# Viictor/vrenderer

Hardware: AMD Instinct MI355X
Metric: shaded Gpixels/s at 8K terrain (higher is better)
Workload: dtype f32

## Files before the change

### vrenderer_amd/csrc/vr_internal.h

```cpp
#pragma once

#include <hip/hip_runtime.h>
#include <hip/hip_ext.h>
#include <stdint.h>
#include <stdlib.h>
#include <string>
#include <vector>

#include "../../include/vrterrain.h"

void vr_set_error(const char* fmt, ...);
#define VR_HIP(expr)                                                                  \
    do {                                                                              \
        hipError_t e__ = (expr);                                                      \
        if (e__ != hipSuccess) {                                                      \
            vr_set_error("%s:%d: %s -> %s", __FILE__, __LINE__, #expr, hipGetErrorString(e__)); \
            return e__ == hipErrorOutOfMemory ? VR_ERR_OUT_OF_MEMORY : VR_ERR_HIP;    \
        }                                                                             \
    } while (0)
#define VR_REQUIRE(cond, msg)                                                         \
    do { if (!(cond)) { vr_set_error("%s:%d: %s", __FILE__, __LINE__, msg); return VR_ERR_INVALID_ARGUMENT; } } while (0)

constexpr int kGrid = 32;
constexpr int kSide = kGrid + 1;
// ... 122 lines not shown
    uint2* d_ranges = nullptr;
    int ranges_tiles = 0;
    enum { RANGES_NONE = 0, RANGES_CLEAN, RANGES_VALID, RANGES_DIRTY };
    int ranges_state = RANGES_NONE;
    int ranges_rank = 0, ranges_world = 1;
    bool emissive_zero = false;
    bool escaped = false;
    uint8_t* d_region = nullptr;
    int region_tiles = 0;
    int region_fill = 0;
    bool clear_pending = false;
    bool cleared_once = false;
};
int vr_gbuffer_materialise(vr_gbuffer* g, hipStream_t s);
constexpr uint32_t kRegionSpec = 1u, kRegionClear = 2u;
int vr_gbuffer_region_prepare(vr_gbuffer* g, hipStream_t s, uint8_t** out);
struct PlaneHints {
    const uint8_t* region;
    uint32_t spec_const;
    int emissive_zero;
    int tiles32_x;
};
int vr_gbuffer_plane_hints(vr_gbuffer* g, hipStream_t s, PlaneHints* out);
uint32_t vr_specular_constant(const vr_context* c);
inline void vr_gbuffer_touch(vr_gbuffer* g) { if (g->ranges_state == vr_gbuffer::RANGES_VALID) g->ranges_state = vr_gbuffer::RANGES_DIRTY; }
int vr_gbuffer_ranges_prepare(vr_gbuffer* g, hipStream_t s);

struct vr_image {
    vr_context* ctx;
    int w, h;
    void* data;
    bool owned;
    size_t capacity_bytes;
    hipEvent_t ev_written = nullptr, ev_read_done = nullptr;
    bool read_pending = false;
};

struct vr_ldr_image {
    vr_context* ctx;
    int w, h;
    void* data;
    bool owned;
    size_t capacity_bytes;
};

constexpr int kGeoSets = 3;
struct GeoSet {
    uint32_t* d_node_ids = nullptr;
    vr_instance* d_instances = nullptr;
    uint32_t* d_counters = nullptr;
    uint32_t* d_sel_scratch = nullptr;
    DevVert* d_verts = nullptr;
    uint64_t* d_rect = nullptr;
    uint4* d_recs = nullptr;
    uint32_t* d_hard_list = nullptr;
    HardTriRec* d_hard_tris = nullptr;
    uint32_t* d_hard_first = nullptr;
    uint32_t* d_tile_count = nullptr;
    uint32_t* d_tile_offset = nullptr;
    uint32_t* d_tile_cursor = nullptr;
    int32_t* d_tile_order = nullptr;
    TileEntry* d_bin_entries = nullptr;
    int scratch_tiles = 0;
    int last_tiles = 0;
    hipEvent_t ev_geo_done = nullptr, ev_raster_done = nullptr;
    hipEvent_t raster_done = nullptr;
    uint64_t raster_done_epoch = 0;
    bool raster_recorded = false, have_selection = false;
    bool geo_recorded = false;
    hipEvent_t ev_sel_read = nullptr;
    bool sel_read_pending = false;
    bool main_waited = false;
    hipStream_t main_wait_stream = nullptr;
    hipStream_t stream = nullptr;
    bool main_dep_pending = false;
    bool status_pending = false;
    bool prepared = false;
    uint64_t prep_serial = 0;
    vr_view prep_view; vr_render_params prep_rp; int prep_w = 0, prep_h = 0, prep_rank = 0, prep_world = 0, prep_tile_shift = 0;
};

struct vr_terrain {
    vr_context* ctx;
    vr_terrain_params p;
    int num_lods;
    float lod_ranges[VR_MAX_LODS];
    DevTex height, albedo;
    uint8_t* d_height = nullptr; uint8_t* d_albedo = nullptr;
    uint64_t bytes_textures = 0, bytes_scratch = 0;
    uint32_t extra_vert_cap = 0, hard_cap = 0;
    size_t bin_capacity = 0;
    int cap_instances = 0;
    uint32_t* h_status = nullptr;
    uint32_t* d_status = nullptr;
    uint32_t high_water = 0;
    size_t bin_high_water = 0, bin_want = 0;
    int sticky_error = 0;
    uint32_t sticky_count = 0;
    GeoSet sets[kGeoSets];
    int cur = 0;
    uint64_t prep_counter = 0;
    hipStream_t geo_streams[2] = { nullptr, nullptr };
    unsigned geo_turn = 0;
    float2* d_node_heights = nullptr;
    uchar2* d_minmax = nullptr;
    bool height_loaded = false;
// ... 54 lines not shown
```

### vrenderer_amd/csrc/vr_raster.hip

```cpp
#include "vr_internal.h"
#include "vr_tex_dev.h"
#include "vr_deferred_dev.h"
#include "vr_experiments.h"
#include <type_traits>

#include <stdlib.h>
#include <string.h>

struct VertexArgs {
    float w2v[16], v2c[16];
    float cam_x, cam_z;
    float lod_ranges[VR_MAX_LODS];
    float morph_start, world_size, max_height;
    float vp_x, vp_y, vp_w, vp_h;
};

struct RasterArgs {
    int w, h;
    int vx0, vy0, vx1, vy1;
    int rtx, rty;
    int tile_shift;
    int mirrored;
    int world, rank;
    uint32_t world_magic;
    int depth_only, assume_cleared;
    int wireframe;
    float world_size, inv_world_size;
    int ws_pow2;
    float lod_w, lod_h, max_level_f;
    uint32_t bin_capacity;
    uint32_t extra_vert_base, extra_vert_cap, hard_cap;
    float vp_x, vp_y, vp_w, vp_h;
};

enum { C_COUNT = 0, C_FLAGS = 1, C_HARDTRIS = 2, C_XVERTS = 3, C_HARDLIST = 4, C_BINTOTAL = 5, C_CLASS0 = 8 };


__device__ __forceinline__ void snap_vertex(DevVert& v, float vp_x, float vp_y, float vp_w, float vp_h)
{
    float iw = 1.0f / v.cw;
    float nx = v.cx * iw, ny = v.cy * iw;
    float sx = (nx * 0.5f + 0.5f) * vp_w + vp_x;
    float sy = (ny * -0.5f + 0.5f) * vp_h + vp_y;
    float fx = floorf(sx * 256.0f + 0.5f), fy = floorf(sy * 256.0f + 0.5f);
    fx = vr_min(vr_max(fx, -1.0e9f), 1.0e9f); fy = vr_min(vr_max(fy, -1.0e9f), 1.0e9f);
    v.X = (int32_t)fx; v.Y = (int32_t)fy;
    v.z = v.cz * iw; v.iw = iw;
}

__global__ __launch_bounds__(256) void k_vertex(VertexArgs a, DevTex hm, const vr_instance* __restrict__ inst,
                                                 uint32_t* __restrict__ counters, DevVert* __restrict__ verts)
{
    VR_GEOMETRY_PRIORITY();
    if (blockIdx.x == 0 && threadIdx.x < 14 && (threadIdx.x < 4 || threadIdx.x >= 6)) counters[2 + threadIdx.x] = 0u;
    __shared__ float r8[256];
    __shared__ uint32_t s_qoff[kMaxLevels];
    r8[threadIdx.x] = (float)threadIdx.x / 255.0f;
    if (threadIdx.x < kMaxLevels) s_qoff[threadIdx.x] = hm.qoff[threadIdx.x];
    __syncthreads();
    const uint32_t total = counters[C_COUNT] * (uint32_t)kVertsPerInst;
    for (uint32_t v = blockIdx.x * blockDim.x + threadIdx.x; v < total; v += gridDim.x * blockDim.x) {
        const uint32_t i = v / kVertsPerInst, r = v - i * kVertsPerInst;
        const int vz = (int)(r / kSide), vx = (int)(r - (uint32_t)vz * kSide);
        const float* M = inst[i].transform;
        const float half = (float)(kGrid / 2), gs = (float)kGrid;
        const float p0 = (float)(vx - kGrid / 2) / half, p1 = 0.0f, p2 = (float)(vz - kGrid / 2) / half;
        float world[4];
#pragma unroll
        for (int k = 0; k < 3; k++) world[k] = ((M[k * 4 + 0] * p0 + M[k * 4 + 1] * p1) + M[k * 4 + 2] * p2) + M[k * 4 + 3] * 1.0f;
        world[3] = 1.0f;
        const float dx = world[0] - a.cam_x, dz = world[2] - a.cam_z;
        const float distance = sqrtf(dx * dx + dz * dz);
        const float gridExtents = 2.0f * sqrtf((M[0] * M[0] + M[4] * M[4]) + M[8] * M[8]);
        int lod = gridExtents > 0.0f ? (int)((__float_as_uint(gridExtents) >> 23) & 255u) - 127 : 0;
        lod = lod < 0 ? 0 : (lod > 11 ? 11 : lod);
        const float start = a.lod_ranges[lod] * a.morph_start, end = a.lod_ranges[lod];
        const float delta = end - start;
        const float morphK = vr_saturate((distance - start) / delta);
        const float gp0 = (p0 + 1.0f) * 0.5f, gp1 = (p2 + 1.0f) * 0.5f;
        {
            float q = gp0 * gs * 0.5f; float fr = (q - floorf(q)) * 2.0f / gs;
            world[0] = world[0] - fr * gridExtents * morphK;
            q = gp1 * gs * 0.5f; fr = (q - floorf(q)) * 2.0f / gs;
            world[2] = world[2] - fr * gridExtents * morphK;
        }
        const float halfSize = a.world_size * 0.5f;
        const float u = (world[0] + halfSize) / a.world_size, w_ = (world[2] + halfSize) / a.world_size;
        {
            const LodSplit ls = vr_lod_split(hm.levels, 0.1f);
            const int l1 = min(ls.l0 + 1, hm.levels - 1);
            const int w0 = max(1, hm.w0 >> ls.l0), h0 = max(1, hm.h0 >> ls.l0), w1 = max(1, hm.w0 >> l1), h1 = max(1, hm.h0 >> l1);
            const QuadTap t0 = quad_tap(w0, h0, u, w_), t1 = quad_tap(w1, h1, u, w_);
            const uint32_t e0 = hm.quad[s_qoff[ls.l0] + t0.idx], e1 = hm.quad[s_qoff[l1] + t1.idx];
            const float s0 = quad_filter(e0, t0, r8), s1 = quad_filter(e1, t1, r8);
            const float hv = ls.f > 0.0f ? __builtin_fmaf(s1 - s0, ls.f, s0) : s0;
            world[1] = hv * a.max_height;
        }
        float viewPos[4], clip[4];
#pragma unroll
        for (int j = 0; j < 4; j++) viewPos[j] = ((world[0] * a.w2v[0 * 4 + j] + world[1] * a.w2v[1 * 4 + j]) + world[2] * a.w2v[2 * 4 + j]) + world[3] * a.w2v[3 * 4 + j];
#pragma unroll
        for (int j = 0; j < 4; j++) clip[j] = ((viewPos[0] * a.v2c[0 * 4 + j] + viewPos[1] * a.v2c[1 * 4 + j]) + viewPos[2] * a.v2c[2 * 4 + j]) + viewPos[3] * a.v2c[3 * 4 + j];
        DevVert o;
        o.cx = clip[0]; o.cy = clip[1]; o.cz = clip[2]; o.cw = clip[3];
        o.wx = world[0]; o.wz = world[2];
        o.pad0 = 0; o.pad1 = 0;
        if (o.cw > 0.0f) snap_vertex(o, a.vp_x, a.vp_y, a.vp_w, a.vp_h);
// ... 141 lines not shown
    uint32_t flags;
    int bx0, by0, bx1, by1;
};
__device__ __forceinline__ int64_t edge_eval(int32_t A, int32_t B, int64_t C, int32_t PX, int32_t PY);
__device__ __forceinline__ int64_t rec_c(const uint4& g);
__device__ __forceinline__ uint32_t order_of(uint32_t key);
__device__ __forceinline__ TriCov load_tri_cov(const uint4* __restrict__ rp)
{
    const uint4 g0 = rp[0], g1 = rp[1], g2 = rp[2], g3 = rp[3], g4 = rp[4];
    TriCov c;
    c.A0 = (int32_t)g0.x; c.B0 = (int32_t)g0.y; c.A1 = (int32_t)g1.x; c.B1 = (int32_t)g1.y; c.A2 = (int32_t)g2.x; c.B2 = (int32_t)g2.y;
    c.C0 = rec_c(g0); c.C1 = rec_c(g1); c.C2 = rec_c(g2);
    c.z0 = __uint_as_float(g3.x); c.zx = __uint_as_float(g3.y); c.zy = __uint_as_float(g3.z); c.flags = g3.w;
    c.bx0 = (int)(g4.x & 0xffffu); c.by0 = (int)(g4.x >> 16); c.bx1 = (int)(g4.y & 0xffffu); c.by1 = (int)(g4.y >> 16);
    return c;
}
__device__ __forceinline__ void write_tile_entry(const RasterArgs& a, TileEntry* __restrict__ dst, const TriCov& c, uint32_t key, int tx, int ty)
{
    const int tile = 1 << a.tile_shift;
    const int ox = tx << a.tile_shift, oy = ty << a.tile_shift;
    const int32_t PX0 = ox * 256 + 128, PY0 = oy * 256 + 128;
    const int64_t e0 = edge_eval(c.A0, c.B0, c.C0, PX0, PY0), e1 = edge_eval(c.A1, c.B1, c.C1, PX0, PY0), e2 = edge_eval(c.A2, c.B2, c.C2, PX0, PY0);
    const int lx0 = max(ox, a.vx0), ly0 = max(oy, a.vy0), lx1 = min(ox + tile - 1, a.vx1), ly1 = min(oy + tile - 1, a.vy1);
    const int x0 = max(c.bx0, lx0) - ox, y0 = max(c.by0, ly0) - oy, x1 = min(c.bx1, lx1) - ox, y1 = min(c.by1, ly1) - oy;
    const bool valid = x0 <= x1 && y0 <= y1;
    bool fits32 = (c.flags & 8u) != 0u;
    if (!fits32) {
        const int64_t lim = (int64_t)1 << 30;
        const int64_t w0 = (int64_t)(kRasterTile + 8) * 256 * (llabs((int64_t)c.A0) + llabs((int64_t)c.B0));
        const int64_t w1 = (int64_t)(kRasterTile + 8) * 256 * (llabs((int64_t)c.A1) + llabs((int64_t)c.B1));
        const int64_t w2 = (int64_t)(kRasterTile + 8) * 256 * (llabs((int64_t)c.A2) + llabs((int64_t)c.B2));
        fits32 = llabs(e0) + w0 < lim && llabs(e1) + w1 < lim && llabs(e2) + w2 < lim;
    }
#define MUL256(v) ((uint32_t)(v) * 256u)
    uint4* __restrict__ q = reinterpret_cast<uint4*>(dst);
    q[0] = make_uint4((uint32_t)e0, (uint32_t)e1, (uint32_t)e2, MUL256(c.A0));
    q[1] = make_uint4(MUL256(c.B0), MUL256(c.A1), MUL256(c.B1), MUL256(c.A2));
    q[2] = make_uint4(MUL256(c.B2), valid ? ((uint32_t)x0 | ((uint32_t)y0 << 8) | ((uint32_t)x1 << 16) | ((uint32_t)y1 << 24)) : 0u,
                      __float_as_uint(c.z0), __float_as_uint(c.zx));
    q[3] = make_uint4(__float_as_uint(c.zy), ((uint32_t)(ox - c.bx0) & 0xffffu) | ((uint32_t)(oy - c.by0) << 16), order_of(key),
                      (c.flags & 7u) | (fits32 ? kTeFits32 : 0u) | (valid ? kTeValid : 0u) | ((c.flags & 8u) ? kTeSmall : 0u));
#undef MUL256
}

template <bool FILL>
__device__ __forceinline__ void bin_rect(const RasterArgs& a, uint64_t r, uint32_t entry, uint32_t* __restrict__ counters_or_cursor,
                                         TileEntry* __restrict__ entries, const TriCov& cov)
{
    const int tx0 = (int)(r & 0xffffu), ty0 = (int)((r >> 16) & 0xffffu), tx1 = (int)((r >> 32) & 0xffffu), ty1 = (int)((r >> 48) & 0xffffu);
    const bool live = r != ~0ull;
    const bool single = live && tx0 == tx1 && ty0 == ty1;
    const int tile = (single && tile_owned(a, tx0, ty0)) ? ty0 * a.rtx + tx0 : -1;
    const int lane = (int)(threadIdx.x & 63u);
    unsigned long long todo = __ballot(tile >= 0);
    while (todo) {
        const int lead = __ffsll((long long)todo) - 1;
        const int t = __builtin_amdgcn_readlane(tile, lead);
        const unsigned long long same = __ballot(tile == t);
        const uint32_t n = (uint32_t)__popcll(same);
        uint32_t base = 0;
        if (lane == lead) base = atomicAdd(&counters_or_cursor[t], n);
        if (FILL) {
            base = (uint32_t)__builtin_amdgcn_readlane((int)base, lead);
            if (tile == t) {
                const uint32_t pos = base + (uint32_t)__popcll(same & ((1ull << lane) - 1ull));
                if (pos < a.bin_capacity) write_tile_entry(a, entries + pos, cov, entry, tx0, ty0);
            }
        }
        todo &= ~same;
    }
    if (live && !single) {
        if (FILL && tx1 - tx0 <= 1 && ty1 - ty0 <= 1) {
            uint32_t pos[4]; bool use[4];
#pragma unroll
            for (int q = 0; q < 4; q++) {
                const int tx = tx0 + (q & 1), ty = ty0 + (q >> 1);
                use[q] = tx <= tx1 && ty <= ty1 && tile_owned(a, tx, ty);
                pos[q] = use[q] ? atomicAdd(&counters_or_cursor[ty * a.rtx + tx], 1u) : 0u;
            }
#pragma unroll
            for (int q = 0; q < 4; q++) if (use[q] && pos[q] < a.bin_capacity) write_tile_entry(a, entries + pos[q], cov, entry, tx0 + (q & 1), ty0 + (q >> 1));
        } else
        for (int ty = ty0; ty <= ty1; ty++)
            for (int tx = tx0; tx <= tx1; tx++)
                if (tile_owned(a, tx, ty)) {
                    const uint32_t pos = atomicAdd(&counters_or_cursor[ty * a.rtx + tx], 1u);
                    if (FILL && pos < a.bin_capacity) write_tile_entry(a, entries + pos, cov, entry, tx, ty);
                }
    }
}

struct ClipVert { float c[4]; float wx, wz; };

__device__ int clip_poly(ClipVert* poly, int n, int plane)
{
    ClipVert out[12];
    float d[12];
    int m = 0;
    for (int i = 0; i < n; i++) {
        const float* c = poly[i].c;
        switch (plane) {
        case 0: d[i] = c[2]; break;
        case 1: d[i] = kGuardBand * c[3] + c[0]; break;
        case 2: d[i] = kGuardBand * c[3] - c[0]; break;
        case 3: d[i] = kGuardBand * c[3] + c[1]; break;
        default: d[i] = kGuardBand * c[3] - c[1]; break;
        }
    }
    for (int i = 0; i < n; i++) {
        const int j = (i + 1 == n) ? 0 : i + 1;
        const bool ini = d[i] >= 0.0f, inj = d[j] >= 0.0f;
        if (ini) out[m++] = poly[i];
        if (ini != inj) {
            const ClipVert& va = ini ? poly[i] : poly[j];
            const ClipVert& vb = ini ? poly[j] : poly[i];
            const float da = ini ? d[i] : d[j], db = ini ? d[j] : d[i];
            const float tt = da / (da - db);
            ClipVert nv;
            for (int k = 0; k < 4; k++) nv.c[k] = va.c[k] + (vb.c[k] - va.c[k]) * tt;
            nv.wx = va.wx + (vb.wx - va.wx) * tt;
            nv.wz = va.wz + (vb.wz - va.wz) * tt;
            out[m++] = nv;
        }
// ... 98 lines not shown
        for (int c = 0; c < kScanClasses; c++) cc[c] += cl == c ? 1u : 0u;
    }
    uint32_t incl = s, ci[kScanClasses];
#pragma unroll
    for (int c = 0; c < kScanClasses; c++) ci[c] = cc[c];
#pragma unroll
    for (int d = 1; d < 64; d <<= 1) {
        const uint32_t v = (uint32_t)__shfl_up((int)incl, d);
        if (lane >= d) incl += v;
#pragma unroll
        for (int c = 0; c < kScanClasses; c++) { const uint32_t w = (uint32_t)__shfl_up((int)ci[c], d); if (lane >= d) ci[c] += w; }
    }
    if (lane == 63) {
        s_wsum[wave] = incl;
#pragma unroll
        for (int c = 0; c < kScanClasses; c++) s_cls[c * NW + wave] = ci[c];
    }
    __syncthreads();
    if (tid <= kScanClasses) {
        uint32_t* __restrict__ w = tid < kScanClasses ? &s_cls[tid * NW] : s_wsum;
        const uint32_t w0 = w[0], w1 = w[1], w2 = w[2], w3 = w[3], total = (w0 + w1) + (w2 + w3);
        uint32_t base = total ? atomicAdd(&counters[tid < kScanClasses ? C_CLASS0 + tid : C_BINTOTAL], total) : 0u;
        if (tid == kScanClasses) { if (base + total > capacity) atomicOr(&counters[C_FLAGS], 2u); }
        else base += (uint32_t)tid * (uint32_t)n_tiles;
        w[0] = base; w[1] = base + w0; w[2] = base + (w0 + w1); w[3] = base + (w0 + w1) + w2;
    }
    __syncthreads();
    uint32_t run = s_wsum[wave] + (incl - s);
    uint32_t slot[kScanClasses];
#pragma unroll
    for (int c = 0; c < kScanClasses; c++) slot[c] = s_cls[c * NW + wave] + (ci[c] - cc[c]);
#pragma unroll
    for (int j = 0; j < kScanPerThread; j++) {
        if (t[j] < 0) continue;
        tile_offset[t[j]] = run; tile_cursor[t[j]] = run; run += cnt[j]; tile_count[t[j]] = 0u;
        const int cl = scan_class(cnt[j]);
        uint32_t pos = 0u;
#pragma unroll
        for (int c = 0; c < kScanClasses; c++) if (cl == c) { pos = slot[c]; slot[c] = pos + 1u; }
        order[pos] = t[j];
    }
}
template <typename OP, typename CP>
__device__ __forceinline__ int tile_of_block(int i, OP order, CP class_totals, int stride)
{
    int c = 0;
#pragma unroll
    for (int q = 0; q < kScanClasses - 1; q++) { const int k = (int)class_totals[q]; if (c == q && i >= k) { i -= k; c = q + 1; } }
    return order[(size_t)c * stride + i];
}

__global__ __launch_bounds__(256) void k_setup(RasterArgs a, const DevVert* __restrict__ verts, uint32_t* __restrict__ counters,
                                                uint64_t* __restrict__ rect, uint32_t* __restrict__ hard_list,
                                                uint32_t* __restrict__ tile_count, uint4* __restrict__ recs)
{
    VR_GEOMETRY_PRIORITY();
    const uint32_t total = counters[C_COUNT] * (uint32_t)kTrisPerInst;
    for (uint32_t tri = blockIdx.x * blockDim.x + threadIdx.x; tri < total; tri += gridDim.x * blockDim.x) {
        uint32_t i0, i1, i2;
        regular_tri_indices(tri, i0, i1, i2);
        const float4 c0 = *reinterpret_cast<const float4*>(&verts[i0].cx);
        const float4 c1 = *reinterpret_cast<const float4*>(&verts[i1].cx);
        const float4 c2 = *reinterpret_cast<const float4*>(&verts[i2].cx);
        const bool out_l = (c0.x < -c0.w) && (c1.x < -c1.w) && (c2.x < -c2.w);
        const bool out_r = (c0.x > c0.w) && (c1.x > c1.w) && (c2.x > c2.w);
        const bool out_b = (c0.y < -c0.w) && (c1.y < -c1.w) && (c2.y < -c2.w);
        const bool out_t = (c0.y > c0.w) && (c1.y > c1.w) && (c2.y > c2.w);
        const bool out_n = (c0.z < 0.0f) && (c1.z < 0.0f) && (c2.z < 0.0f);
        const bool out_f = (c0.z > c0.w) && (c1.z > c1.w) && (c2.z > c2.w);
        uint64_t r = ~0ull;
        if (!(out_l || out_r || out_b || out_t || out_n || out_f)) {
            const bool need_near = (c0.z < 0.0f) || (c1.z < 0.0f) || (c2.z < 0.0f);
            const float g0 = kGuardBand * c0.w, g1 = kGuardBand * c1.w, g2 = kGuardBand * c2.w;
            const bool need_guard = (c0.x < -g0) || (c0.x > g0) || (c0.y < -g0) || (c0.y > g0)
                                 || (c1.x < -g1) || (c1.x > g1) || (c1.y < -g1) || (c1.y > g1)
                                 || (c2.x < -g2) || (c2.x > g2) || (c2.y < -g2) || (c2.y > g2);
            if (need_near || need_guard) {
                const uint32_t slot = atomicAdd(&counters[C_HARDLIST], 1u);
                if (slot < a.hard_cap) hard_list[slot] = tri; else atomicOr(&counters[C_FLAGS], 2u);
            } else {
                r = triangle_rect(a, load_sv(verts, i0), load_sv(verts, i1), load_sv(verts, i2), recs + (size_t)tri * kRecGroups);
            }
        }
        bin_rect<false>(a, r, 0u, tile_count, nullptr, TriCov());
        rect[tri] = r;
    }
}

__global__ __launch_bounds__(64) void k_clip(RasterArgs a, DevVert* __restrict__ verts, uint32_t* __restrict__ counters,
                                              const uint32_t* __restrict__ hard_list, HardTriRec* __restrict__ hard_tris,
                                              uint32_t* __restrict__ hard_first, uint32_t* __restrict__ tile_count,
                                              uint4* __restrict__ hard_recs)
{
    VR_GEOMETRY_PRIORITY();
    const uint32_t n_hard = min(counters[C_HARDLIST], a.hard_cap);
    clip_hard_list(a, verts, counters, hard_list, hard_tris, hard_first, tile_count, hard_recs, blockIdx.x * blockDim.x + threadIdx.x, n_hard,
                   gridDim.x * blockDim.x);
}

__global__ __launch_bounds__(256) void k_fill(RasterArgs a, const uint32_t* __restrict__ counters, const uint64_t* __restrict__ rect,
                                               const HardTriRec* __restrict__ hard_tris, const uint4* __restrict__ recs, uint32_t rec_hard_base,
                                               uint32_t* __restrict__ tile_cursor, TileEntry* __restrict__ entries, uint32_t* __restrict__ status)
{
    VR_GEOMETRY_PRIORITY();
    if (blockIdx.x == 0 && threadIdx.x < 8) { __hip_atomic_store(&status[threadIdx.x], counters[threadIdx.x], __ATOMIC_RELAXED, __HIP_MEMORY_SCOPE_SYSTEM); }
    const uint32_t n_reg = counters[C_COUNT] * (uint32_t)kTrisPerInst;
    const uint32_t n_hard = min(counters[C_HARDTRIS], a.hard_cap * 4u);
    for (uint32_t i = blockIdx.x * blockDim.x + threadIdx.x; i < n_reg + n_hard; i += gridDim.x * blockDim.x) {
        uint64_t r; uint32_t entry; size_t rec;
        if (i < n_reg) { r = rect[i]; entry = i << 4; rec = i; }
        else {
            const HardTriRec h = hard_tris[i - n_reg];
            r = (uint64_t)h.rect_lo | ((uint64_t)h.rect_hi << 32); entry = h.order_key;
            rec = (size_t)rec_hard_base + (i - n_reg);
        }
        TriCov cov = TriCov();
        if (r != ~0ull) cov = load_tri_cov(recs + rec * kRecGroups);
        bin_rect<true>(a, r, entry, tile_cursor, entries, cov);
    }
}

template <typename HF>
__device__ __forceinline__ size_t rec_index(uint32_t key, HF hard_first, uint32_t rec_hard_base)
{
    const uint32_t tri = key >> 4;
    if (key & 1u) return (size_t)rec_hard_base + hard_first[tri] + ((key >> 1) & 7u);
    return (size_t)tri;
}

template <typename HF>
__device__ __forceinline__ void entry_vertices(uint32_t key, const HardTriRec* __restrict__ hard_tris, HF hard_first,
                                               uint32_t& i0, uint32_t& i1, uint32_t& i2)
{
    const uint32_t tri = key >> 4;
    if (key & 1u) {
        const HardTriRec rec = hard_tris[hard_first[tri] + ((key >> 1) & 7u)];
        i0 = rec.v0; i1 = rec.v1; i2 = rec.v2;
    } else {
        regular_tri_indices(tri, i0, i1, i2);
    }
}

__device__ __forceinline__ int64_t edge_eval(int32_t A, int32_t B, int64_t C, int32_t PX, int32_t PY)
{
    return (int64_t)A * PX + ((int64_t)B * PY + C);
}
__device__ __forceinline__ int64_t rec_c(const uint4& g) { return (int64_t)(((uint64_t)g.w << 32) | (uint64_t)g.z); }

struct Attr { float wx, wz, dwxdx, dwzdx, dwxdy, dwzdy; };

__device__ __forceinline__ float div_ws(const RasterArgs& a, float s)
{
    return a.ws_pow2 ? s * a.inv_world_size : s / a.world_size;
}
__device__ __forceinline__ float to_uv(const RasterArgs& a, float x) { return div_ws(a, x + a.world_size * 0.5f); }

struct Axis { int i; float f; };
__device__ __forceinline__ Axis tap_axis(int n, float t)
{
    const float x = __builtin_fmaf(t, (float)n, -0.5f);
    float xf = floorf(x);
    Axis r; r.f = x - xf;
    r.i = (int)vr_clampf(xf, -1.0f, (float)n);
// ... 811 lines not shown
static int launch_geometry(vr_terrain* t, GeoSet& g, GeoSet* selection_from, const vr_view* view, const vr_render_params* rp,
                           const RasterArgs& a, const PartTables* pt)
{
    vr_context* ctx = t->ctx;
    g.stream = t->geo_streams[t->geo_turn++ & 1u];
    g.main_waited = false;
    hipStream_t s = ctx->stream, gs = g.stream;
    if (!ctx->async_geometry) {
        VR_HIP(hipEventRecord(t->ev_main_dep, s));
        g.main_dep_pending = true;
    }
    if (g.geo_recorded) VR_HIP(hipStreamWaitEvent(gs, g.ev_geo_done, 0));
    if (g.sel_read_pending) { VR_HIP(hipStreamWaitEvent(gs, g.ev_sel_read, 0)); g.sel_read_pending = false; }
    if (g.raster_recorded && (g.raster_done_epoch == 0 || g.raster_done_epoch == ctx->ev_epoch)) VR_HIP(hipStreamWaitEvent(gs, g.raster_done, 0));
    if (g.main_dep_pending) { VR_HIP(hipStreamWaitEvent(gs, t->ev_main_dep, 0)); g.main_dep_pending = false; }
    int rc;
    if (selection_from == nullptr) {
        if ((rc = vr_select_launch(t, g, view, rp->max_height, gs))) return rc;
    } else if (selection_from != &g) {
        VR_HIP(hipEventRecord(t->ev_sel_copy, selection_from->stream));
        VR_HIP(hipStreamWaitEvent(gs, t->ev_sel_copy, 0));
        VR_HIP(hipMemcpyAsync(g.d_node_ids, selection_from->d_node_ids, (size_t)t->p.max_instances * sizeof(uint32_t), hipMemcpyDeviceToDevice, gs));
        VR_HIP(hipMemcpyAsync(g.d_instances, selection_from->d_instances, (size_t)t->p.max_instances * sizeof(vr_instance), hipMemcpyDeviceToDevice, gs));
        VR_HIP(hipMemcpyAsync(g.d_counters, selection_from->d_counters, 2 * sizeof(uint32_t), hipMemcpyDeviceToDevice, gs));
        VR_HIP(hipEventRecord(selection_from->ev_sel_read, gs));
        selection_from->sel_read_pending = true;
        g.have_selection = true;
    }
    const int n_tiles = a.rtx * a.rty;
    if (n_tiles > g.scratch_tiles) {
        VR_HIP(hipStreamSynchronize(gs));
        VR_HIP(hipStreamSynchronize(s));
        (void)hipFree(g.d_tile_count); (void)hipFree(g.d_tile_offset); (void)hipFree(g.d_tile_cursor); (void)hipFree(g.d_tile_order);
        g.d_tile_count = g.d_tile_offset = g.d_tile_cursor = nullptr; g.d_tile_order = nullptr; g.scratch_tiles = 0;
        VR_HIP(hipMalloc(&g.d_tile_count, sizeof(uint32_t) * n_tiles));
        VR_HIP(hipMalloc(&g.d_tile_offset, sizeof(uint32_t) * n_tiles));
        VR_HIP(hipMalloc(&g.d_tile_cursor, sizeof(uint32_t) * n_tiles));
        VR_HIP(hipMalloc(&g.d_tile_order, sizeof(int32_t) * n_tiles * kScanClasses));
        VR_HIP(hipMemsetAsync(g.d_tile_count, 0, sizeof(uint32_t) * n_tiles, gs));
        VR_HIP(hipMemsetAsync(g.d_tile_cursor, 0, sizeof(uint32_t) * n_tiles, gs));
        VR_HIP(hipMemsetAsync(g.d_tile_offset, 0, sizeof(uint32_t) * n_tiles, gs));
        g.scratch_tiles = n_tiles;
    }
    g.last_tiles = n_tiles;
    VertexArgs va;
    for (int i = 0; i < 16; i++) { va.w2v[i] = view->world_to_view[i]; va.v2c[i] = view->view_to_clip[i]; }
    va.cam_x = view->camera_pos[0]; va.cam_z = view->camera_pos[2];
    for (int i = 0; i < VR_MAX_LODS; i++) va.lod_ranges[i] = t->lod_ranges[i];
    va.morph_start = t->p.morph_start; va.world_size = t->p.world_size; va.max_height = rp->max_height;
    va.vp_x = a.vp_x; va.vp_y = a.vp_y; va.vp_w = a.vp_w; va.vp_h = a.vp_h;
    { VrKernelScope ks(ctx, VR_K_VERTEX, gs);
    hipLaunchKernelGGL(k_vertex, dim3(kGridVertex), dim3(256), 0, gs, va, t->height, g.d_instances, g.d_counters, g.d_verts); }
    { VrKernelScope ks(ctx, VR_K_SETUP, gs);
    hipLaunchKernelGGL(k_setup, dim3(kGridSetup), dim3(256), 0, gs, a, g.d_verts, g.d_counters, g.d_rect, g.d_hard_list, g.d_tile_count, g.d_recs); }
    { VrKernelScope ks(ctx, VR_K_CLIP, gs);
    hipLaunchKernelGGL(k_clip, dim3(64), dim3(64), 0, gs, a, g.d_verts, g.d_counters, g.d_hard_list, g.d_hard_tris, g.d_hard_first, g.d_tile_count,
                       g.d_recs + (size_t)t->cap_instances * kTrisPerInst * kRecGroups); }
    { VrKernelScope ks(ctx, VR_K_SCAN, gs);
    const bool whole = pt == nullptr;
    const int n_scan = whole ? n_tiles : pt->num_raster_tiles;
    if (n_scan > 0)
        hipLaunchKernelGGL(k_scan, dim3((n_scan + kScanPerGroup - 1) / kScanPerGroup), dim3(256), 0, gs, n_tiles, g.d_tile_count, g.d_tile_offset,
                           g.d_tile_cursor, g.d_counters, a.bin_capacity, whole ? (const int32_t*)nullptr : (const int32_t*)pt->d_raster_tiles, n_scan,
                           g.d_tile_order); }
    { VrKernelScope ks(ctx, VR_K_FILL, gs);
    hipLaunchKernelGGL(k_fill, dim3(kGridFill), dim3(256), 0, gs, a, g.d_counters, g.d_rect, g.d_hard_tris, (const uint4*)g.d_recs,
                       (uint32_t)t->cap_instances * (uint32_t)kTrisPerInst, g.d_tile_cursor, g.d_bin_entries, t->d_status + (size_t)(&g - t->sets) * 8); }
    g.status_pending = true;
    VR_HIP(hipEventRecord(g.ev_geo_done, gs));
    g.geo_recorded = true;
    VR_HIP(hipGetLastError());
    return VR_OK;
}

typedef decltype(&k_raster<false, 32, RM_GENERIC>) raster_kernel_t;
template <int TILE>
static raster_kernel_t pick_raster(bool wire, bool fast, bool depth, bool ranges, bool noemi)
{
    if (wire) return k_raster<true, TILE, RM_GENERIC>;
    if (fast) return ranges ? (noemi ? k_raster<false, TILE, RM_FAST, true, true> : k_raster<false, TILE, RM_FAST, true, false>)
                            : (noemi ? k_raster<false, TILE, RM_FAST, false, true> : k_raster<false, TILE, RM_FAST, false, false>);
    return depth ? k_raster<false, TILE, RM_DEPTH> : k_raster<false, TILE, RM_GENERIC>;
}

static bool prepared_matches(const GeoSet& g, const vr_view* view, const vr_render_params* rp, int w, int h, const RasterArgs& a)
{
    return memcmp(&g.prep_view, view, sizeof(vr_view)) == 0 && g.prep_rp.max_height == rp->max_height && g.prep_rp.depth_only == rp->depth_only
        && !g.prep_rp.wireframe == !rp->wireframe && g.prep_w == w && g.prep_h == h && g.prep_rank == a.rank && g.prep_world == a.world
        && g.prep_tile_shift == a.tile_shift;
}

static int check_render_inputs(vr_terrain* t, const vr_view* view, vr_gbuffer* gb, const vr_render_params* rp)
{
    VR_REQUIRE(t && view && gb && rp, "NULL argument");
    VR_REQUIRE(!view->reverse_depth, "reverse depth is not supported (the reference disables it, Renderer.cpp:221)");
    VR_REQUIRE(view->viewport_w > 0 && view->viewport_h > 0 && view->viewport_w <= 16384 && view->viewport_h <= 16384, "bad viewport");
    VR_REQUIRE(gb->ctx == t->ctx, "G-buffer and terrain belong to different contexts");
    return VR_OK;
}

extern "C" VR_API int vr_terrain_prepare(vr_terrain* t, const vr_view* view, vr_gbuffer* gb, const vr_render_params* rp,
                                          const vr_partition* part)
{
    int rc = check_render_inputs(t, view, gb, rp);
    if (rc) return rc;
    VR_REQUIRE(!rp->lock_view, "vr_terrain_prepare builds a new selection; it cannot be combined with lock_view");
    VR_HIP(hipSetDevice(t->ctx->device));
    if ((rc = vr_terrain_poll(t, false))) return rc;
    RasterArgs a;
    if ((rc = make_raster_args(t, view, rp, gb->w, gb->h, part, a))) return rc;
    if ((rc = vr_terrain_reserve_bins(t, (size_t)a.rtx * a.rty / (size_t)(a.world > 1 ? a.world : 1)))) return rc;
    a.bin_capacity = (uint32_t)t->bin_capacity;
    const PartTables* pt = nullptr;
    if (a.world > 1 && (rc = vr_partition_tables(t->ctx, gb->w, gb->h, part, &pt))) return rc;
    for (GeoSet& p : t->sets)
        if (p.prepared && prepared_matches(p, view, rp, gb->w, gb->h, a)) return VR_OK;
    GeoSet& g = t->sets[vr_terrain_pick_set(t)];
    g.prepared = false;
    if (t->raster_begin_recorded && (t->start_hint_epoch == 0 || t->start_hint_epoch == t->ctx->ev_epoch))
// ... 175 lines not shown
```

### vrenderer_amd/csrc/vr_select.hip

```cpp
#include "vr_internal.h"
#include "vr_experiments.h"

#include <math.h>
#include <string.h>
#include <stdlib.h>

constexpr int kSelThreads = 256;
constexpr int kFrontierCap = 4096;
constexpr int kFrontLds = 1536;
constexpr int kSelectedCap = 4096;
constexpr int kRankChunk = 1024;
constexpr int kSelScratchWords = 2 * (kFrontierCap - kFrontLds) + kSelectedCap;

struct SelectArgs {
    float cam[3];
    float planes[6][4];
    float range2[VR_MAX_LODS];
    float loc[3];
    float half_w, half_h;
    int num_lods;
    int max_instances;
    int cap_instances;
    int height_loaded;
    float max_height;
// ... 355 lines not shown
        a.loc[0] = t->p.location[0] + x * t->p.surface_size; a.loc[1] = t->p.location[1] + 0.0f; a.loc[2] = t->p.location[2] + y * t->p.surface_size;
    }
    float2* out = t->d_node_heights + (size_t)surf * nodes;
    int rx0 = 0, ry0 = 0, leaf = 0;
    if (dyadic_root(t, a.loc, &rx0, &ry0, &leaf)) {
        if (!t->d_minmax) VR_HIP(hipMalloc(&t->d_minmax, nodes * sizeof(uchar2)));
        for (int d = t->num_lods; d >= 0; d--) {
            const uint32_t n = 1u << d;
            const uint64_t base = ((((uint64_t)1 << (2 * d)) - 1) / 3), cells = (uint64_t)n * n, blocks = (cells + 255) / 256;
            const unsigned grid = (unsigned)(blocks > 16384 ? 16384 : blocks);
            if (d == t->num_lods)
                hipLaunchKernelGGL(k_minmax_leaf, dim3(grid), dim3(256), 0, t->ctx->stream, (const uint8_t*)t->d_height, t->height.w0, rx0, ry0, n, leaf,
                                   t->d_minmax + base, out + base);
            else
                hipLaunchKernelGGL(k_minmax_up, dim3(grid), dim3(256), 0, t->ctx->stream,
                                   (const uchar2*)(t->d_minmax + ((((uint64_t)1 << (2 * (d + 1))) - 1) / 3)), n, t->d_minmax + base, out + base);
        }
        continue;
    }
    for (int d = 0; d <= t->num_lods; d++) {
        a.depth = d;
        const uint64_t n = (uint64_t)1 << (2 * d);
        const double per_node = ((double)t->p.surface_size * t->texel_size[0]) * ((double)t->p.surface_size * t->texel_size[1]) / (double)n;
        if (per_node >= 512.0 && n <= (1u << 20))
            hipLaunchKernelGGL(k_node_heights_block, dim3((unsigned)n), dim3(256), 0, t->ctx->stream, a, t->d_height, out);
        else {
            const uint64_t blocks = (n + 255) / 256;
            hipLaunchKernelGGL(k_node_heights_thread, dim3((unsigned)(blocks > 8192 ? 8192 : blocks)), dim3(256), 0, t->ctx->stream, a,
                               t->d_height, out);
        }
    }
    }
    VR_HIP(hipGetLastError());
    VR_HIP(hipEventRecord(t->ev_main_dep, t->ctx->stream));
    for (GeoSet& g : t->sets) g.main_dep_pending = true;
    t->height_loaded = true;
    return VR_OK;
}

extern "C" VR_API int vr_terrain_download_node_heights(vr_terrain* t, uint32_t first, uint32_t count, float* out)
{
    VR_REQUIRE(t && out && t->d_node_heights, "node heights have not been computed");
    const uint64_t nodes = ((((uint64_t)1 << (2 * (t->num_lods + 1))) - 1) / 3) * (uint64_t)(t->surfaces_per_side * t->surfaces_per_side);
    VR_REQUIRE((uint64_t)first + count <= nodes, "node id range out of bounds");
    VR_HIP(hipSetDevice(t->ctx->device));
    VR_HIP(hipStreamSynchronize(t->ctx->stream));
    VR_HIP(hipMemcpy(out, t->d_node_heights + first, (size_t)count * sizeof(float2), hipMemcpyDeviceToHost));
    return VR_OK;
}

static void free_scratch(vr_terrain* t)
{
    for (GeoSet& g : t->sets) {
        (void)hipFree(g.d_verts); (void)hipFree(g.d_rect); (void)hipFree(g.d_recs); (void)hipFree(g.d_hard_first); (void)hipFree(g.d_bin_entries);
        g.d_verts = nullptr; g.d_rect = nullptr; g.d_recs = nullptr; g.d_hard_first = nullptr; g.d_bin_entries = nullptr;
    }
}
static int alloc_scratch(vr_terrain* t, int cap)
{
    free_scratch(t);
    const size_t mi = (size_t)cap, fixed = (size_t)t->p.max_instances * (sizeof(uint32_t) + sizeof(vr_instance)) + 64 * sizeof(uint32_t)
                    + kSelScratchWords * sizeof(uint32_t) + (size_t)t->hard_cap * (sizeof(uint32_t) + 4 * sizeof(HardTriRec));
    t->bytes_scratch = (uint64_t)fixed * kGeoSets;
    t->bin_capacity = ((size_t)1 << 20) * ((mi + 1023) / 1024);
    if (const char* e = getenv("VR_SCRATCH_INITIAL_BINS")) { const long v = atol(e); if (v >= 1024) t->bin_capacity = (size_t)v; }
    if (t->bin_want > t->bin_capacity) t->bin_capacity = t->bin_want;
#define VR_ALLOC(ptr, bytes) do { hipError_t e_ = hipMalloc(&(ptr), (bytes)); if (e_ != hipSuccess) { \
        vr_set_error("hipMalloc(%zu) failed: %s", (size_t)(bytes), hipGetErrorString(e_)); return VR_ERR_OUT_OF_MEMORY; } \
        t->bytes_scratch += (uint64_t)(bytes); } while (0)
    for (GeoSet& g : t->sets) {
        VR_ALLOC(g.d_verts, (mi * kVertsPerInst + t->extra_vert_cap) * sizeof(DevVert));
        VR_ALLOC(g.d_rect, mi * kTrisPerInst * sizeof(uint64_t));
        VR_ALLOC(g.d_recs, (mi * kTrisPerInst + (size_t)t->hard_cap * 4) * kRecGroups * sizeof(uint4));
        VR_ALLOC(g.d_hard_first, mi * kTrisPerInst * sizeof(uint32_t));
        VR_ALLOC(g.d_bin_entries, t->bin_capacity * sizeof(TileEntry));
        g.prepared = false;
    }
#undef VR_ALLOC
    t->cap_instances = cap;
    return VR_OK;
}

int vr_terrain_reserve_bins(vr_terrain* t, size_t tiles)
{
    const size_t est = tiles * 8;
    if (est <= t->bin_capacity) return VR_OK;
    size_t b = t->bin_capacity ? t->bin_capacity : ((size_t)1 << 20);
    while (b < est) b *= 2;
    t->bin_want = b;
    VR_HIP(hipSetDevice(t->ctx->device));
    for (hipStream_t gs : t->geo_streams) VR_HIP(hipStreamSynchronize(gs));
    VR_HIP(hipStreamSynchronize(t->ctx->stream));
    return alloc_scratch(t, t->cap_instances);
}

int vr_terrain_poll(vr_terrain* t, bool report)
{
    uint32_t seen = 0;
    for (int i = 0; i < kGeoSets; i++) {
        GeoSet& g = t->sets[i];
        if (!g.status_pending || !g.geo_recorded || hipEventQuery(g.ev_geo_done) != hipSuccess) continue;
        g.status_pending = false;
        const volatile uint32_t* st = t->h_status + i * 8;
        const uint32_t flags = st[1], wanted = st[6];
        if (wanted > seen) seen = wanted;
        if ((size_t)st[5] > t->bin_high_water) t->bin_high_water = (size_t)st[5];
        if (flags & 1u) { t->sticky_error = VR_ERR_TOO_MANY_INSTANCES; t->sticky_count = wanted; }
        else if (flags & 6u) { if (!t->sticky_error) t->sticky_error = VR_ERR_OVERFLOW; t->sticky_count = wanted; }
    }
    if (seen > t->high_water) t->high_water = seen;
    const int max_i = t->p.max_instances;
    const bool grow_nodes = t->cap_instances < max_i && (size_t)t->high_water * 2 > (size_t)t->cap_instances;
    const bool grow_bins = t->bin_high_water * 2 > t->bin_capacity;
    if (grow_nodes || grow_bins) {
        int want = t->cap_instances;
        while (want < max_i && (size_t)t->high_water * 2 > (size_t)want) want *= 2;
        if (want > max_i) want = max_i;
        if (grow_bins) { size_t b = t->bin_capacity; while (b < t->bin_high_water * 2) b *= 2; t->bin_want = b; }
        VR_HIP(hipSetDevice(t->ctx->device));
        for (hipStream_t gs : t->geo_streams) VR_HIP(hipStreamSynchronize(gs));
        VR_HIP(hipStreamSynchronize(t->ctx->stream));
        const int had = t->cap_instances;
        int rc = alloc_scratch(t, want);
        if (rc) {
            t->bin_want = 0;
// ... 268 lines not shown
```

Baseline: 79.02.

## Compact live triangles in setup and restructure wave-level bin atomics

Setup now appends each surviving triangle's index to a compacted live list, using a wave-aggregated atomic counter, and writes rect only for live triangles. Fill iterates over that list instead of every triangle slot, so culled triangles no longer cost a thread. bin_rect also changes: lanes first find their group leader and rank, then one atomic per group is issued outside the loop. In exchange it adds an extra atomic, a scatter write and an indirection load per triangle, plus a new buffer and counter slot.

After: 79.29, median of 6. No clear change (+0.3%).

```diff
diff --git a/vrenderer_amd/csrc/vr_internal.h b/vrenderer_amd/csrc/vr_internal.h
--- a/vrenderer_amd/csrc/vr_internal.h
+++ b/vrenderer_amd/csrc/vr_internal.h
@@ -198,6 +198,7 @@
     uint32_t* d_sel_scratch = nullptr;
     DevVert* d_verts = nullptr;
     uint64_t* d_rect = nullptr;
+    uint32_t* d_live_list = nullptr;
     uint4* d_recs = nullptr;
     uint32_t* d_hard_list = nullptr;
     HardTriRec* d_hard_tris = nullptr;
diff --git a/vrenderer_amd/csrc/vr_raster.hip b/vrenderer_amd/csrc/vr_raster.hip
--- a/vrenderer_amd/csrc/vr_raster.hip
+++ b/vrenderer_amd/csrc/vr_raster.hip
@@ -33,7 +33,7 @@
     float vp_x, vp_y, vp_w, vp_h;
 };
 
-enum { C_COUNT = 0, C_FLAGS = 1, C_HARDTRIS = 2, C_XVERTS = 3, C_HARDLIST = 4, C_BINTOTAL = 5, C_CLASS0 = 8 };
+enum { C_COUNT = 0, C_FLAGS = 1, C_HARDTRIS = 2, C_XVERTS = 3, C_HARDLIST = 4, C_BINTOTAL = 5, C_CLASS0 = 8, C_LIVE = 16 };
 
 
 __device__ __forceinline__ void snap_vertex(DevVert& v, float vp_x, float vp_y, float vp_w, float vp_h)
@@ -52,7 +52,7 @@
                                                  uint32_t* __restrict__ counters, DevVert* __restrict__ verts)
 {
     VR_GEOMETRY_PRIORITY();
-    if (blockIdx.x == 0 && threadIdx.x < 14 && (threadIdx.x < 4 || threadIdx.x >= 6)) counters[2 + threadIdx.x] = 0u;
+    if (blockIdx.x == 0 && threadIdx.x < 15 && (threadIdx.x < 4 || threadIdx.x >= 6)) counters[2 + threadIdx.x] = 0u;
     __shared__ float r8[256];
     __shared__ uint32_t s_qoff[kMaxLevels];
     r8[threadIdx.x] = (float)threadIdx.x / 255.0f;
@@ -300,23 +300,25 @@
     const bool single = live && tx0 == tx1 && ty0 == ty1;
     const int tile = (single && tile_owned(a, tx0, ty0)) ? ty0 * a.rtx + tx0 : -1;
     const int lane = (int)(threadIdx.x & 63u);
+    int my_lead = lane; uint32_t group_n = 0, group_rank = 0;
     unsigned long long todo = __ballot(tile >= 0);
     while (todo) {
         const int lead = __ffsll((long long)todo) - 1;
         const int t = __builtin_amdgcn_readlane(tile, lead);
         const unsigned long long same = __ballot(tile == t);
-        const uint32_t n = (uint32_t)__popcll(same);
+        if (tile == t) { my_lead = lead; group_n = (uint32_t)__popcll(same); group_rank = (uint32_t)__popcll(same & ((1ull << lane) - 1ull)); }
+        todo &= ~same;
+    }
+    const bool leads = tile >= 0 && my_lead == lane;
+    if (FILL) {
         uint32_t base = 0;
-        if (lane == lead) base = atomicAdd(&counters_or_cursor[t], n);
-        if (FILL) {
-            base = (uint32_t)__builtin_amdgcn_readlane((int)base, lead);
-            if (tile == t) {
-                const uint32_t pos = base + (uint32_t)__popcll(same & ((1ull << lane) - 1ull));
-                if (pos < a.bin_capacity) write_tile_entry(a, entries + pos, cov, entry, tx0, ty0);
-            }
-        }
-        todo &= ~same;
-    }
+        if (leads) base = atomicAdd(&counters_or_cursor[tile], group_n);
+        base = (uint32_t)__shfl((int)base, my_lead);
+        if (tile >= 0) {
+            const uint32_t pos = base + group_rank;
+            if (pos < a.bin_capacity) write_tile_entry(a, entries + pos, cov, entry, tx0, ty0);
+        }
+    } else if (leads) atomicAdd(&counters_or_cursor[tile], group_n);
     if (live && !single) {
         if (FILL && tx1 - tx0 <= 1 && ty1 - ty0 <= 1) {
             uint32_t pos[4]; bool use[4];
@@ -521,9 +523,10 @@
 
 __global__ __launch_bounds__(256) void k_setup(RasterArgs a, const DevVert* __restrict__ verts, uint32_t* __restrict__ counters,
                                                 uint64_t* __restrict__ rect, uint32_t* __restrict__ hard_list,
-                                                uint32_t* __restrict__ tile_count, uint4* __restrict__ recs)
+                                                uint32_t* __restrict__ tile_count, uint4* __restrict__ recs, uint32_t* __restrict__ live_list)
 {
     VR_GEOMETRY_PRIORITY();
+    const int lane = (int)(threadIdx.x & 63u);
     const uint32_t total = counters[C_COUNT] * (uint32_t)kTrisPerInst;
     for (uint32_t tri = blockIdx.x * blockDim.x + threadIdx.x; tri < total; tri += gridDim.x * blockDim.x) {
         uint32_t i0, i1, i2;
@@ -551,8 +554,16 @@
                 r = triangle_rect(a, load_sv(verts, i0), load_sv(verts, i1), load_sv(verts, i2), recs + (size_t)tri * kRecGroups);
             }
         }
+        const bool live = r != ~0ull;
+        const unsigned long long lm = __ballot(live);
+        uint32_t base = 0;
+        const int lead = __ffsll((long long)lm) - 1;
+        if (lane == lead) base = atomicAdd(&counters[C_LIVE], (uint32_t)__popcll(lm));
         bin_rect<false>(a, r, 0u, tile_count, nullptr, TriCov());
-        rect[tri] = r;
+        if (lm) {
+            base = (uint32_t)__builtin_amdgcn_readlane((int)base, lead);
+            if (live) { live_list[base + (uint32_t)__popcll(lm & ((1ull << lane) - 1ull))] = tri; rect[tri] = r; }
+        }
     }
 }
 
@@ -568,16 +579,17 @@
 }
 
 __global__ __launch_bounds__(256) void k_fill(RasterArgs a, const uint32_t* __restrict__ counters, const uint64_t* __restrict__ rect,
-                                               const HardTriRec* __restrict__ hard_tris, const uint4* __restrict__ recs, uint32_t rec_hard_base,
+                                               const uint32_t* __restrict__ live_list, const HardTriRec* __restrict__ hard_tris,
+                                               const uint4* __restrict__ recs, uint32_t rec_hard_base,
                                                uint32_t* __restrict__ tile_cursor, TileEntry* __restrict__ entries, uint32_t* __restrict__ status)
 {
     VR_GEOMETRY_PRIORITY();
     if (blockIdx.x == 0 && threadIdx.x < 8) { __hip_atomic_store(&status[threadIdx.x], counters[threadIdx.x], __ATOMIC_RELAXED, __HIP_MEMORY_SCOPE_SYSTEM); }
-    const uint32_t n_reg = counters[C_COUNT] * (uint32_t)kTrisPerInst;
+    const uint32_t n_reg = counters[C_LIVE];
     const uint32_t n_hard = min(counters[C_HARDTRIS], a.hard_cap * 4u);
     for (uint32_t i = blockIdx.x * blockDim.x + threadIdx.x; i < n_reg + n_hard; i += gridDim.x * blockDim.x) {
         uint64_t r; uint32_t entry; size_t rec;
-        if (i < n_reg) { r = rect[i]; entry = i << 4; rec = i; }
+        if (i < n_reg) { const uint32_t tri = live_list[i]; r = rect[tri]; entry = tri << 4; rec = tri; }
         else {
             const HardTriRec h = hard_tris[i - n_reg];
             r = (uint64_t)h.rect_lo | ((uint64_t)h.rect_hi << 32); entry = h.order_key;
@@ -1495,7 +1507,8 @@
     { VrKernelScope ks(ctx, VR_K_VERTEX, gs);
     hipLaunchKernelGGL(k_vertex, dim3(kGridVertex), dim3(256), 0, gs, va, t->height, g.d_instances, g.d_counters, g.d_verts); }
     { VrKernelScope ks(ctx, VR_K_SETUP, gs);
-    hipLaunchKernelGGL(k_setup, dim3(kGridSetup), dim3(256), 0, gs, a, g.d_verts, g.d_counters, g.d_rect, g.d_hard_list, g.d_tile_count, g.d_recs); }
+    hipLaunchKernelGGL(k_setup, dim3(kGridSetup), dim3(256), 0, gs, a, g.d_verts, g.d_counters, g.d_rect, g.d_hard_list, g.d_tile_count, g.d_recs,
+                       g.d_live_list); }
     { VrKernelScope ks(ctx, VR_K_CLIP, gs);
     hipLaunchKernelGGL(k_clip, dim3(64), dim3(64), 0, gs, a, g.d_verts, g.d_counters, g.d_hard_list, g.d_hard_tris, g.d_hard_first, g.d_tile_count,
                        g.d_recs + (size_t)t->cap_instances * kTrisPerInst * kRecGroups); }
@@ -1507,7 +1520,7 @@
                            g.d_tile_cursor, g.d_counters, a.bin_capacity, whole ? (const int32_t*)nullptr : (const int32_t*)pt->d_raster_tiles, n_scan,
                            g.d_tile_order); }
     { VrKernelScope ks(ctx, VR_K_FILL, gs);
-    hipLaunchKernelGGL(k_fill, dim3(kGridFill), dim3(256), 0, gs, a, g.d_counters, g.d_rect, g.d_hard_tris, (const uint4*)g.d_recs,
+    hipLaunchKernelGGL(k_fill, dim3(kGridFill), dim3(256), 0, gs, a, g.d_counters, g.d_rect, g.d_live_list, g.d_hard_tris, (const uint4*)g.d_recs,
                        (uint32_t)t->cap_instances * (uint32_t)kTrisPerInst, g.d_tile_cursor, g.d_bin_entries, t->d_status + (size_t)(&g - t->sets) * 8); }
     g.status_pending = true;
     VR_HIP(hipEventRecord(g.ev_geo_done, gs));
diff --git a/vrenderer_amd/csrc/vr_select.hip b/vrenderer_amd/csrc/vr_select.hip
--- a/vrenderer_amd/csrc/vr_select.hip
+++ b/vrenderer_amd/csrc/vr_select.hip
@@ -431,8 +431,8 @@
 static void free_scratch(vr_terrain* t)
 {
     for (GeoSet& g : t->sets) {
-        (void)hipFree(g.d_verts); (void)hipFree(g.d_rect); (void)hipFree(g.d_recs); (void)hipFree(g.d_hard_first); (void)hipFree(g.d_bin_entries);
-        g.d_verts = nullptr; g.d_rect = nullptr; g.d_recs = nullptr; g.d_hard_first = nullptr; g.d_bin_entries = nullptr;
+        (void)hipFree(g.d_verts); (void)hipFree(g.d_rect); (void)hipFree(g.d_live_list); (void)hipFree(g.d_recs); (void)hipFree(g.d_hard_first); (void)hipFree(g.d_bin_entries);
+        g.d_verts = nullptr; g.d_rect = nullptr; g.d_live_list = nullptr; g.d_recs = nullptr; g.d_hard_first = nullptr; g.d_bin_entries = nullptr;
     }
 }
 static int alloc_scratch(vr_terrain* t, int cap)
@@ -450,6 +450,7 @@
     for (GeoSet& g : t->sets) {
         VR_ALLOC(g.d_verts, (mi * kVertsPerInst + t->extra_vert_cap) * sizeof(DevVert));
         VR_ALLOC(g.d_rect, mi * kTrisPerInst * sizeof(uint64_t));
+        VR_ALLOC(g.d_live_list, mi * kTrisPerInst * sizeof(uint32_t));
         VR_ALLOC(g.d_recs, (mi * kTrisPerInst + (size_t)t->hard_cap * 4) * kRecGroups * sizeof(uint4));
         VR_ALLOC(g.d_hard_first, mi * kTrisPerInst * sizeof(uint32_t));
         VR_ALLOC(g.d_bin_entries, t->bin_capacity * sizeof(TileEntry));
```
